# LaurenYTaylor/jsrl-CORL

Measured on AMD Instinct MI355X. Metric: IQL gradient-steps/sec at batch=256 (D4RL obs/act dims), higher is better.
Workload: dtype f32; 1 GPU; IQL step on synthetic buffer (obs=17, act=6, 1000000 rows), batch=256 per GPU; global_batch=256, parallelism=single, prepare_rehearsal_steps=1111

## Files before the change

### jsrl-corl_amd/csrc/iqlhip.hip

```cpp
#include "iqlhip_kernels.h"
#include "iqlhip_lb_kernels.h"

#include <dlfcn.h>

#include <time.h>

#include <algorithm>
#include <cstdarg>
#include <cstdio>
#include <cstdlib>
#include <cstring>
#include <string>
#include <type_traits>
#include <vector>

#define GRAPH_STEPS IQLHIP_GRAPH_STEPS
static const int kChunkSizes[] = {GRAPH_STEPS, 16, 4, 2, 1};

static thread_local std::string g_err;

static int fail(int code, const char* fmt, ...) {
  char buf[512];
  va_list ap;
  va_start(ap, fmt);
// ... 221 lines not shown
}

extern "C" int64_t iqlhip_row_stride(int32_t S, int32_t A) { return up(2 * (int64_t)S + A + 2, 4); }

static int xld_host(int k0) { int k0p = (k0 + 3) & ~3; return ((k0p + 29) / 32) * 32 + 2; }

extern "C" int iqlhip_destroy(iqlhip_ctx* c);
extern "C" int iqlhip_xch_shutdown(iqlhip_ctx* c);

static int create_impl(iqlhip_ctx* c, const iqlhip_dims* dims, const iqlhip_hyper* hyper, int device) {
  c->dims = *dims;
  c->hyper = *hyper;
  c->device = device;
  iqlhip_arena_layout(dims, &c->L);
  const int MB = dims->max_batch, A = dims->action_dim;
  c->n_chunk_max = (MB + CHUNK_ROWS - 1) / CHUNK_ROWS;
  c->n_rt_max = (MB + RT_ROWS - 1) / RT_ROWS;
  c->sc.max_batch = MB;
  auto dalloc = [&](float** p, size_t nfloat) -> hipError_t {
    hipError_t e = hipMalloc((void**)p, nfloat * sizeof(float));
    if (e != hipSuccess) return e;
    return hipMemset(*p, 0, nfloat * sizeof(float));
  };
  HIPCHK(dalloc(&c->sc.h0, (size_t)4 * MB * HID));
  HIPCHK(dalloc(&c->sc.h1, (size_t)4 * MB * HID));
  HIPCHK(dalloc(&c->sc.heads, (size_t)MB * HEAD_LD + (size_t)NSPLIT * MB * A));
  c->row_ld = iqlhip_row_stride(dims->state_dim, A);
  HIPCHK(dalloc(&c->xb, (size_t)MB * c->row_ld));
  HIPCHK(dalloc(&c->xb2, (size_t)MB * c->row_ld));
  HIPCHK(hipHostMalloc((void**)&c->losses_host, 4 * sizeof(float), hipHostMallocDefault));
  HIPCHK(hipHostMalloc((void**)&c->on_row_pin, (size_t)c->row_ld * sizeof(float), hipHostMallocDefault));
  HIPCHK(hipHostMalloc((void**)&c->on_idx_pin, (size_t)MB * sizeof(long long), hipHostMallocDefault));
  HIPCHK(hipHostMalloc((void**)&c->on_loss_pin, 4 * sizeof(float), hipHostMallocDefault));
  HIPCHK(hipHostMalloc((void**)&c->done_pin, 8 * sizeof(unsigned long long), hipHostMallocDefault));
  memset(c->done_pin, 0, 8 * sizeof(unsigned long long));
  HIPCHK(hipHostMalloc((void**)&c->on_act_pin, (size_t)(IQLHIP_MAX_INPUT + IQLHIP_MAX_ACTION) * sizeof(float), hipHostMallocDefault));
  c->act_cap = std::max(MB, IQLHIP_ACT_ROWS);
  HIPCHK(dalloc(&c->xb_act, (size_t)c->act_cap * c->row_ld));
  HIPCHK(dalloc(&c->heads_act, (size_t)c->act_cap * A * NSPLIT));
  HIPCHK(hipMalloc((void**)&c->drop_bits, (size_t)4 * MB * 8 * sizeof(unsigned)));
  HIPCHK(hipMemset(c->drop_bits, 0xFF, (size_t)4 * MB * 8 * sizeof(unsigned)));
  HIPCHK(dalloc(&c->sc.slab_a, (size_t)c->n_chunk_max * c->L.n_params));
  size_t sb = 0;
  for (int n = 0; n < 4; ++n) {
    c->sc.slab_b_off[n] = (long long)sb;
    sb += (size_t)c->n_rt_max * ((size_t)HID * c->L.net[n].k_in + HID);
  }
  HIPCHK(dalloc(&c->sc.slab_b, sb));
// ... 1688 lines not shown
    if (which == 1 || which == 3 || which == 4 || which == 5) launch_bwd(c, p, st);
    if (which == 2 || which == 3) launch_upd(c, u, st);
  }
  c->lb_bwd_part = 0;
  HIPCHK(hipEventRecord(e1, st));
  HIPCHK(hipEventSynchronize(e1));
  float ms = 0.f;
  HIPCHK(hipEventElapsedTime(&ms, e0, e1));
  *avg_us = ms * 1e3f / repeat;
  (void)hipEventDestroy(e0);
  (void)hipEventDestroy(e1);
  return IQLHIP_OK;
}

extern "C" int iqlhip_debug_read(iqlhip_ctx* c, const char* name, float* host_out, int64_t max_floats, int64_t* n_out,
                                 void* stream) {
  if (!c || !name || !host_out) return fail(IQLHIP_EINVAL, "NULL argument");
  hipStream_t st = (hipStream_t)stream;
  const float* src = nullptr;
  int64_t n = 0;
  const int MB = c->dims.max_batch;
  if (!strcmp(name, "h0")) { src = c->sc.h0; n = (int64_t)4 * MB * HID; }
  else if (!strcmp(name, "h1")) { src = c->sc.h1; n = (int64_t)4 * MB * HID; }
  else if (!strcmp(name, "heads")) { src = c->sc.heads; n = (int64_t)MB * HEAD_LD + (int64_t)NSPLIT * MB * c->dims.action_dim; }
  else if (!strcmp(name, "loss_parts")) { src = c->sc.loss_parts; n = 4 * 64; }
  else if (!strcmp(name, "drop_bits")) { src = (const float*)c->drop_bits; n = (int64_t)2 * MB * 8; }
  else if (!strcmp(name, "stamps")) {
    if (!c->stamps) return fail(IQLHIP_EINVAL, "library built without -DIQL_STAMPS");
    src = (const float*)c->stamps; n = 4096 * 16 * 2;
  }
  else if (!strcmp(name, "grads")) {
    return fail(IQLHIP_EINVAL, "use iqlhip_forward_backward to obtain the flat gradient");
  } else return fail(IQLHIP_EINVAL, "unknown scratch array '%s'", name);
  if (n > max_floats) n = max_floats;
  HIPCHK(hipMemcpyAsync(host_out, src, (size_t)n * sizeof(float), hipMemcpyDeviceToHost, st));
  HIPCHK(hipStreamSynchronize(st));
  if (n_out) *n_out = n;
  return IQLHIP_OK;
}


template <class T> struct Section { size_t off = 0; };
struct Staging {
  char* dev = nullptr;
  char* pin = nullptr;
  size_t bytes = 0;
// ... 538 lines not shown
```

### jsrl-corl_amd/csrc/iqlhip_bwd_body.inc

```
  RT_ENTRY();
  const int bid = blockIdx.x;
  const int x = bid & 7;
  const int h_S = (int)(q_dims & 255u), h_A = (int)((q_dims >> 8) & 63u), h_pol = (int)((q_dims >> 14) & 1u);
  const int h_ld = (int)(q_ldB & 1023u), h_rows = (int)(q_ldB >> 10);
  const int h_MB = (int)(q_mbc & 0xFFFFu), n_chunk = (int)(q_mbc >> 16);
  const int n_rt = (int)(q_rts & 1023u), h_spb = (int)(q_rts >> 10);
  unsigned kpf[8] = {0, 0, 0, 0, 0, 0, 0, 0};
  if constexpr (!MULTI && KPF) {
    const unsigned long long ka = (unsigned long long)(uintptr_t)__builtin_amdgcn_kernarg_segment_ptr();
    constexpr unsigned KA_P = 56;
    const unsigned o_net = KA_P + (unsigned)offsetof(StepParams, net) + (unsigned)sizeof(NetPtrs) * (unsigned)(x & 3);
    const unsigned o_go = KA_P + (unsigned)offsetof(StepParams, go) + (unsigned)sizeof(NetGrad) * (unsigned)(x & 3);
    const unsigned o_t0 = (KA_P + (unsigned)offsetof(StepParams, log_std)) & ~63u;
    static_assert(KA_P + sizeof(StepParams) - ((KA_P + offsetof(StepParams, log_std)) & ~(size_t)63) <= 256, "kernel-argument tail: more than 4 lines");
    unsigned d0, d1, d2, d3, d4, d5, d6, d7;
    asm volatile(
        "s_load_dword %0, %8, %9\n\ts_load_dword %1, %8, %10\n\ts_load_dword %2, %8, %11\n\t"
        "s_load_dword %3, %8, %12\n\ts_load_dword %4, %8, %13\n\ts_load_dword %5, %8, %14\n\t"
        "s_load_dword %6, %8, %15\n\ts_load_dword %7, %8, %16"
        : "=&s"(d0), "=&s"(d1), "=&s"(d2), "=&s"(d3), "=&s"(d4), "=&s"(d5), "=&s"(d6), "=&s"(d7)
        : "s"(ka), "s"(o_net), "s"(o_net + (unsigned)sizeof(NetPtrs) - 4u), "s"(o_go), "s"(o_go + (unsigned)sizeof(NetGrad) - 4u),
          "s"(o_t0), "s"(o_t0 + 64u), "s"(o_t0 + 128u), "s"(o_t0 + 192u));
    kpf[0] = d0; kpf[1] = d1; kpf[2] = d2; kpf[3] = d3; kpf[4] = d4; kpf[5] = d5; kpf[6] = d6; kpf[7] = d7;
  }
// ... 10 lines not shown
      const int j = q * 6 + (x - (x >> 2));
      if (net == IQLHIP_NET_PI || j >= n_don) return;
      net = IQLHIP_NET_PI;
      local_ = n_a + n_b - n_don + j;
    } else {
      local_ -= 2 * n_e;
      if (net == IQLHIP_NET_PI && local_ >= n_a + n_b - n_don) return;
    }
  }
  const int tid = threadIdx.x, lane = tid & 63, wave = tid >> 6;
  const int l15 = lane & 15, g = lane >> 4;
  const int B = h_rows;
  const int MB = h_MB;
  const ArenaOff ao = arena_off(net, h_S, h_A, h_pol == IQLHIP_POLICY_GAUSSIAN);

  const NetPtrs np = p.net[net];
  const NetGrad go = p.go[net];
  const int D = ao.d;
  const int Dp = (D + 15) & ~15;
  const int DYLD = Dp + 4;
  const float* w2 = q_params + ao.w2;
  const float* H1g = BF16 ? (const float*)((const __bf16*)q_h1 + net * MB * HID) : q_h1 + net * MB * HID;
  const float* H0g = BF16 ? (const float*)((const __bf16*)q_h0 + net * MB * HID) : q_h0 + net * MB * HID;
#define PIN_REST()                                                                                                          \
  do {                                                                                                                      \
    float* sa_ = p.sc.slab_a; float* sb_ = p.sc.slab_b;                                                                     \
    const long long sbo_ = p.sc.slab_b_off[net], npar_ = p.n_params;                                                        \
    PIN_P(np.w1); PIN_P(sa_); PIN_P(sb_);                                                                                   \
    PIN_S(sbo_); PIN_S(npar_); PIN_S(go.w1); PIN_S(go.b1); PIN_S(go.w2); PIN_S(go.b2); PIN_S(go.log_std);                   \
    PIN_S(p.inv_batch); PIN_S(p.hy.iql_tau); PIN_S(p.hy.beta); PIN_S(p.hy.discount); PIN_S(p.hy.exp_adv_max);               \
    if constexpr (!MULTI && KPF)                                                                                            \
      asm volatile("s_waitcnt lgkmcnt(0)" ::"s"(kpf[0]), "s"(kpf[1]), "s"(kpf[2]), "s"(kpf[3]), "s"(kpf[4]), "s"(kpf[5]),   \
                   "s"(kpf[6]), "s"(kpf[7]));                                                                               \
  } while (0)
  if (local_ >= n_a + n_b) return;
  const int local = MULTI ? ((local_ < n_b) ? n_a + local_ : local_ - n_b) : local_;

  extern __shared__ __attribute__((aligned(16))) float smem[];
  STAMP_BASE(p, 2048 * 16);
  STAMP(p, 0);

  if (local < n_a) {
    const int c = local >> 5;
    const int jt = (local >> 2) & 7;
    const int it = local & 3;
    const int j0 = jt * 32, i0 = it * 64;
    const int cbase = c * CHUNK_ROWS;
    float* red = smem;
    const int DYA = Dp + 4;
    float* dYs = red + 4 * 32 * T64_LD;
    float* dLs = dYs + CHUNK_ROWS * DYA;
    float* W2s = dLs + CHUNK_ROWS * DYA;
    float* rsm = W2s + 32 * 32;
    float* wS = rsm + 64;
    const bool designated = (jt == 0 && it == 2);
    const bool loss_block = (jt == 1 && it == 2);
    const bool do_db1 = (it == 0);
    const bool do_dw2 = (D == 1) ? (it == 0) : (it == 1 || it == 3);
    const int tb_own = (it == 3) ? 1 : 0;
    const bool extras = do_db1 || do_dw2;

    const int prow = cbase + tid;
    RowIn in;
    const float lsr = pi_ls_issue_hot(q_params + ao.log_std, q_xb, h_pol, h_A);
    const bool is_pi = (net == IQLHIP_NET_PI);
    row_issue_hot(q_heads, q_xb, h_ld, h_S, h_A, BROW(prow), in);
    const int r8 = tid >> 3, sub = tid & 7;
    const f32x4* hpb = (const f32x4*)(q_heads + MB * HEAD_LD);
    const float* hpf = q_heads + MB * HEAD_LD;
    const float* xbp = q_xb;
    f32x4 php[8];
    float pac[8];
    if (is_pi) {
      const unsigned dd0 = (unsigned)min(sub, h_A - 1);
      const unsigned uA = (unsigned)h_A, uld = (unsigned)h_ld, uS = (unsigned)h_S;
#pragma unroll
      for (int cc = 0; cc < 8; ++cc) {
        const unsigned rowc = (unsigned)BROW(cbase + r8 + 32 * cc);
        php[cc] = *(const f32x4*)(hpf + 4u * (rowc * uA + dd0));
        pac[cc] = xbp[rowc * uld + uS + dd0];
      }
    }
    float w2pre[4];
#pragma unroll
    for (int q = 0; q < 4; ++q) {
      const int ec = min(tid + 256 * q, D * 32 - 1);
      w2pre[q] = w2[(unsigned)((ec >> 5) * HID + j0 + (ec & 31))];
    }
#define AROW(ks) (64 * wave + 16 * ((ks) >> 2) + 4 * g + ((ks) & 3))
    typename Frag2<BF16>::type hh[16];
    typename Frag4<BF16>::type bb[16];
#define HB_LOAD(k0_, k1_)                                                                               \
    _Pragma("unroll") for (int ks = (k0_); ks < (k1_); ++ks) {                                          \
      const unsigned row = (unsigned)BROW(cbase + AROW(ks));                                            \
      hh[ks] = ld2<BF16>(H1g, row * (unsigned)HID + (unsigned)(j0 + 2 * l15));                          \
      bb[ks] = ld4<BF16>(H0g, row * (unsigned)HID + (unsigned)(i0 + 4 * l15));                          \
    }
    HB_LOAD(0, 4);
    PIN_REST();
    float* slab = p.sc.slab_a + (long long)c * p.n_params;
    const float dscale = (net == IQLHIP_NET_PI && p.drop_bits != nullptr) ? p.drop_scale : 1.f;
    STAMP(p, 10);
    {
      const int row = prow;
#pragma unroll
      for (int q = 0; q < 4; ++q) {
        const int e = tid + 256 * q;
        if (e < Dp * 32) W2s[e] = (e < D * 32) ? w2pre[q] : 0.f;
      }
      float lossA = 0.f, lossB = 0.f;
      const PiConst pc = pi_consts_hot(p, h_pol, net, lsr);
      if (!is_pi) {
        float* dyrow = dYs + tid * DYA;
        for (int dd = 0; dd < Dp; ++dd) dyrow[dd] = 0.f;
        if (row < B) row_finish(p, net, in, dyrow, lossA, lossB);
      } else {
        float wrow = 0.f;
        if (row < B) {
// ... 124 lines not shown
      __syncthreads();
      if (tid < D) {
        float u[32], w[32];
#pragma unroll
        for (int k = 0; k < 32; ++k) { u[k] = red[k * 16 + tid]; w[k] = red[k * 16 + 8 + tid]; }
#pragma unroll
        for (int st = 16; st > 0; st >>= 1) {
#pragma unroll
          for (int k = 0; k < 16; ++k) if (k < st) { u[k] += u[k + st]; w[k] += w[k + st]; }
        }
        const float ts = u[0], tl = w[0];
        slab[go.b2 + tid] = ts;
        if (gls) {
          const bool inside = (lsr >= p.hy.log_std_min) && (lsr <= p.hy.log_std_max);
          slab[go.log_std + tid] = inside ? tl * p.inv_batch : 0.f;
        }
      }
    }
    STAMP(p, 2);

    float av[16][2];
    float db1a[2] = {0.f, 0.f};
    float dw2a[2] = {0.f, 0.f};
    if (D == 1) {
      const float w2a = W2s[2 * l15], w2b = W2s[2 * l15 + 1];
#pragma unroll
      for (int ks = 0; ks < 16; ++ks) {
        const float dy = dYs[AROW(ks) * DYA];
        av[ks][0] = ((float)hh[ks][0] > 0.f) ? dy * w2a * dscale : 0.f;
        av[ks][1] = ((float)hh[ks][1] > 0.f) ? dy * w2b * dscale : 0.f;
        if (do_dw2) {
          dw2a[0] = fmaf(dy, (float)hh[ks][0], dw2a[0]);
          dw2a[1] = fmaf(dy, (float)hh[ks][1], dw2a[1]);
        }
      }
    } else {
      f32x4 pre[4][2];
#pragma unroll
      for (int t = 0; t < 4; ++t) { pre[t][0] = (f32x4){0.f, 0.f, 0.f, 0.f}; pre[t][1] = pre[t][0]; }
      if (D <= 8) dh1_mfma<2>(pre, dYs, W2s, DYA, wave, g, l15);
      else if (D <= 16) dh1_mfma<4>(pre, dYs, W2s, DYA, wave, g, l15);
      else dh1_mfma<8>(pre, dYs, W2s, DYA, wave, g, l15);
#pragma unroll
      for (int ks = 0; ks < 16; ++ks) {
        av[ks][0] = ((float)hh[ks][0] > 0.f) ? pre[ks >> 2][0][ks & 3] * dscale : 0.f;
        av[ks][1] = ((float)hh[ks][1] > 0.f) ? pre[ks >> 2][1][ks & 3] * dscale : 0.f;
      }
    }
    if (do_db1) {
#pragma unroll
      for (int ks = 0; ks < 16; ++ks) { db1a[0] += av[ks][0]; db1a[1] += av[ks][1]; }
    }

    f32x4 acc[2][4];
#pragma unroll
    for (int i = 0; i < 2; ++i)
#pragma unroll
      for (int j = 0; j < 4; ++j) acc[i][j] = (f32x4){0.f, 0.f, 0.f, 0.f};
    if constexpr (BF16) {
#pragma unroll
      for (int q = 0; q < 2; ++q) {
        bf16x8 A[2], Bv[4];
#pragma unroll
        for (int ta = 0; ta < 2; ++ta) {
          float t8[8];
#pragma unroll
          for (int e = 0; e < 8; ++e) t8[e] = av[8 * q + e][ta];
          A[ta] = pack8s(t8);
        }
#pragma unroll
        for (int tb = 0; tb < 4; ++tb) {
// ... 6 lines not shown
          for (int tb = 0; tb < 4; ++tb) acc[ta][tb] = MFMA_BF16(A[ta], Bv[tb], acc[ta][tb]);
      }
    } else {
#pragma unroll
      for (int ks = 0; ks < 16; ++ks) {
#pragma unroll
        for (int ta = 0; ta < 2; ++ta)
#pragma unroll
          for (int tb = 0; tb < 4; ++tb) acc[ta][tb] = MFMA16(av[ks][ta], bb[ks][tb], acc[ta][tb]);
      }
    }
    f32x4 acc2[2][2];
#pragma unroll
    for (int i = 0; i < 2; ++i)
#pragma unroll
      for (int j = 0; j < 2; ++j) acc2[i][j] = (f32x4){0.f, 0.f, 0.f, 0.f};
    const int ndt = Dp >> 4;
    if (do_dw2 && D > 1) {
      float ad[16];
#pragma unroll
      for (int ks = 0; ks < 16; ++ks) ad[ks] = dYs[AROW(ks) * DYA + l15];
      float hsel[16];
#pragma unroll
      for (int ks = 0; ks < 16; ++ks) hsel[ks] = tb_own ? (float)hh[ks][1] : (float)hh[ks][0];
#pragma unroll
      for (int ks = 0; ks < 16; ++ks) acc2[0][0] = MFMA16(ad[ks], hsel[ks], acc2[0][0]);
      if (ndt > 1) {
#pragma unroll
        for (int ks = 0; ks < 16; ++ks) ad[ks] = dYs[AROW(ks) * DYA + 16 + l15];
#pragma unroll
        for (int ks = 0; ks < 16; ++ks) acc2[1][0] = MFMA16(ad[ks], hsel[ks], acc2[1][0]);
      }
    }
    STAMP(p, 3);

    float* exA = dLs;
    float* exB = dLs + 1024;
    {
      float* myred = red + wave * 32 * T64_LD;
#pragma unroll
      for (int ta = 0; ta < 2; ++ta)
#pragma unroll
        for (int reg = 0; reg < 4; ++reg) {
          const int jl = 2 * (4 * g + reg) + ta;
          f32x4 v = (f32x4){acc[ta][0][reg], acc[ta][1][reg], acc[ta][2][reg], acc[ta][3][reg]};
          *(f32x4*)(myred + jl * T64_LD + 4 * l15) = v;
        }
// ... 23 lines not shown
        for (int w = 1; w < 4; ++w) s += *(const f32x4*)(red + w * 32 * T64_LD + jl * T64_LD + 4 * i4);
        *(f32x4*)(gw1 + (j0 + jl) * HID + i0 + 4 * i4) = s;
      }
    }
    if (extras) {
      const int e_lo = do_db1 ? 0 : 32;
      const int e_hi = do_dw2 ? (1 + D) * 32 : 32;
      for (int e = tid + e_lo; e < e_hi; e += 256) {
        const int rr = e >> 5, jj = e & 31;
        float s;
        if (rr == 0 || D == 1) {
          float wsum[4];
#pragma unroll
          for (int w = 0; w < 4; ++w) {
            const float* a = exA + (w * 4) * 64 + rr * 32 + jj;
            wsum[w] = (a[0] + a[64]) + (a[128] + a[192]);
          }
          s = (wsum[0] + wsum[1]) + (wsum[2] + wsum[3]);
        } else {
          const float* b = exB + (rr - 1) * 32 + jj;
          s = (b[0] + b[1024]) + (b[2048] + b[3072]);
        }
        if (rr == 0) { if (do_db1) slab[go.b1 + j0 + jj] = s; }
        else if (do_dw2 && (D == 1 || (jj & 1) == tb_own)) slab[go.w2 + (rr - 1) * HID + j0 + jj] = s;
      }
    }
    STAMP(p, 4);
    RT_STAMP(p, 14, rt_entry_);
    RT_STAMP(p, 15, iql_realtime());
    return;
  }
#undef AROW

  {
    const int lb = local - n_a;
    const int rt = lb >> (2 - bsl2);
    int i0 = ((lb & ((4 >> bsl2) - 1)) << bsl2) * 64;
    const int row0 = rt * RT_ROWS;
    const int k0 = ao.k0;
    const int ld = h_ld;
    const int xoff = 0;
    const float* w1 = np.w1;

    float* dH1s = smem;
    __bf16* dH1b = (__bf16*)smem;
    float* red = dH1s + RT_ROWS * H0_LD;
    float* dH0s = red + 4 * 32 * T64_LD;
// ... 15 lines not shown
      const float* hsb = q_heads;
      const unsigned oh = (unsigned)prow8 * (unsigned)HEAD_LD;
      ph[0] = *(const f32x4*)(hsb + (oh + 4u)); ph[1] = *(const f32x4*)(hsb + (oh + 8u)); ph[2] = *(const f32x4*)(hsb + (oh + 12u));
      const float* arow = q_xb + (unsigned)(prow8 * h_ld + h_S);
      const f32x4* hp = (const f32x4*)(q_heads + MB * HEAD_LD + (unsigned)(prow8 * h_A * NSPLIT));
#pragma unroll
      for (int c = 0; c < 4; ++c) {
        php[c] = (f32x4){0.f, 0.f, 0.f, 0.f};
        pac[c] = 0.f;
        if (c == 0 || 8 * c < h_A) {
          const int dd = min(psub + 8 * c, h_A - 1);
          php[c] = hp[dd];
          pac[c] = arow[dd];
        }
      }
    }
    const int j4 = tid & 63;
    const f32x4 w2v = *(const f32x4*)(w2 + 4 * j4);
    f32x4 w2v8[8];
    if (D > 1) {
#pragma unroll
      for (int j = 0; j < 8; ++j) w2v8[j] = *(const f32x4*)(w2 + min(j, D - 1) * HID + 4 * j4);
    }
    typename Frag4<BF16>::type h1v[8];
#define H1V_LOAD(q0_, q1_)                                                                              \
    _Pragma("unroll") for (int q = (q0_); q < (q1_); ++q) {                                             \
      const int f = tid + 256 * q;                                                                      \
      const unsigned row = (unsigned)BROW(row0 + (f >> 6));           \
      h1v[q] = ld4<BF16>(H1g, row * (unsigned)HID + (unsigned)(4 * (f & 63)));                          \
    }
    H1V_LOAD(0, 4);
    constexpr bool FULLB = BF16 && MULTI;
    typename Frag4<BF16>::type bw[FULLB ? 64 : 16];
    typename Frag4<BF16>::type h0v[2];
    const int n_x = RT_ROWS * ld / 4;
    const int x_last = B * ld / 4 - 1;
    PIN_REST();
    const float dscale = (net == IQLHIP_NET_PI && p.drop_bits != nullptr) ? p.drop_scale : 1.f;

    const PiConst pc = pi_consts_hot(p, h_pol, net, lsr);
    if (net == IQLHIP_NET_PI) {
      const float tq = fminf(sum4(ph[1]), sum4(ph[2]));
      const float u = tq - sum4(ph[0]);
      const float w = fminf(expf(p.hy.beta * u), p.hy.exp_adv_max);
      const bool rvalid = (row0 + prl) < B;
      const bool gauss = (h_pol == IQLHIP_POLICY_GAUSSIAN);
#pragma unroll
      for (int c = 0; c < 4; ++c) {
        const int dd = psub + 8 * c;
        if (dd < Dp) {
          float dy = 0.f;
          const int ddc = min(dd, h_A - 1);
          const float ivar = __shfl(pc.ivar, ddc);
          if (rvalid && dd < h_A) {
            const float mu = tanh_via_exp(sum4(php[c]));
            const float diff = pac[c] - mu;
            const float dmu = gauss ? (-(w * diff) * ivar) * p.inv_batch : (-2.f * w * diff) * p.inv_batch;
            dy = dmu * (1.f - mu * mu);
          }
          dYs[prl * DYLD + dd] = dy;
        }
      }
    } else if (tid < RT_ROWS) {
      const int row = row0 + tid;
      float la, lbv;
      float* dyrow = dYs + tid * DYLD;
      for (int dd = 0; dd < Dp; ++dd) dyrow[dd] = 0.f;
      if (row < B) row_finish(p, net, in, dyrow, la, lbv);
    }
    __builtin_amdgcn_sched_barrier(0);
    H1V_LOAD(4, 8);
#undef H1V_LOAD
#pragma unroll
    for (int q = 0; q < 2; ++q) {
      const int f = tid + 256 * q;
      const unsigned row = (unsigned)BROW(row0 + (f >> 4));
      h0v[q] = ld4<BF16>(H0g, row * (unsigned)HID + (unsigned)(i0 + 4 * (f & 15)));
    }
    __builtin_amdgcn_sched_barrier(0);
    __syncthreads();
    STAMP(p, 5);
#define BWB_ROW(ks_) (FULLB ? (32 * ((ks_) >> 3) + 8 * g + ((ks_) & 7)) : (BF16 ? (64 * wave + 32 * ((ks_) >> 3) + 8 * g + ((ks_) & 7)) : (64 * wave + 4 * (ks_) + g)))
#define BWB_COL (FULLB ? (64 * wave + 4 * l15) : (i0 + 4 * l15))
#define BWB_LOAD(ks_) bw[ks_] = ld4<BF16>(w1, (unsigned)(BWB_ROW(ks_) * HID + BWB_COL))

    if (D > 8) {
      f32x4 sacc[8];
#pragma unroll
      for (int q = 0; q < 8; ++q) sacc[q] = (f32x4){0.f, 0.f, 0.f, 0.f};
      f32x4 wv[8], wn[8];
#pragma unroll
      for (int j = 0; j < 8; ++j) wv[j] = w2v8[j];
      for (int d0 = 0; d0 < D; d0 += 8) {
        const bool more = (d0 + 8 < D);
        if (more) {
#pragma unroll
          for (int j = 0; j < 8; ++j) wn[j] = *(const f32x4*)(w2 + min(d0 + 8 + j, D - 1) * HID + 4 * j4);
        }
#pragma unroll
        for (int q = 0; q < 8; ++q) {
          const int rl = (tid + 256 * q) >> 6;
          const f32x4 ya = *(const f32x4*)(dYs + rl * DYLD + d0), yb = *(const f32x4*)(dYs + rl * DYLD + d0 + 4);
#pragma unroll
          for (int j = 0; j < 4; ++j) sacc[q] += ya[j] * wv[j];
#pragma unroll
          for (int j = 0; j < 4; ++j) sacc[q] += yb[j] * wv[4 + j];
        }
        if (more) {
#pragma unroll
          for (int j = 0; j < 8; ++j) wv[j] = wn[j];
        }
      }
#pragma unroll
      for (int q = 0; q < 8; ++q) {
        const int rl = (tid + 256 * q) >> 6;
        f32x4 out;
#pragma unroll
        for (int e = 0; e < 4; ++e) out[e] = ((float)h1v[q][e] > 0.f) ? sacc[q][e] * dscale : 0.f;
        if constexpr (BF16) {
          bf16x4 ob_;
#pragma unroll
          for (int e = 0; e < 4; ++e) ob_[e] = (__bf16)out[e];
          *(bf16x4*)(dH1b + rl * H0B_LD + 4 * j4) = ob_;
        } else {
          *(f32x4*)(dH1s + rl * H0_LD + 4 * j4) = out;
        }
        if constexpr (FULLB) {
#pragma unroll
          for (int e = 0; e < 8; ++e) BWB_LOAD(8 * q + e);
        } else {
          BWB_LOAD(2 * q);
          BWB_LOAD(2 * q + 1);
        }
      }
    } else {
      f32x4 sq[8];
      if (D == 1) {
        float dy1[8];
#pragma unroll
        for (int q = 0; q < 8; ++q) dy1[q] = dYs[((tid + 256 * q) >> 6) * DYLD];
#pragma unroll
// ... 5 lines not shown
#pragma unroll
          for (int qq = 0; qq < 4; ++qq) {
            const int rl = (tid + 256 * (4 * hq + qq)) >> 6;
            ya[qq] = *(const f32x4*)(dYs + rl * DYLD);
            yb[qq] = *(const f32x4*)(dYs + rl * DYLD + 4);
          }
#pragma unroll
          for (int qq = 0; qq < 4; ++qq) {
            f32x4 s = ya[qq][0] * w2v8[0];
#pragma unroll
            for (int j = 1; j < 4; ++j) s += ya[qq][j] * w2v8[j];
#pragma unroll
            for (int j = 0; j < 4; ++j) s += yb[qq][j] * w2v8[4 + j];
            sq[4 * hq + qq] = s;
          }
        }
      }
#pragma unroll
      for (int q = 0; q < 8; ++q) {
        const int rl = (tid + 256 * q) >> 6;
        const f32x4 s = sq[q];
        f32x4 out;
#pragma unroll
        for (int e = 0; e < 4; ++e) out[e] = ((float)h1v[q][e] > 0.f) ? s[e] * dscale : 0.f;
        if constexpr (BF16) {
          bf16x4 ob_;
#pragma unroll
          for (int e = 0; e < 4; ++e) ob_[e] = (__bf16)out[e];
          *(bf16x4*)(dH1b + rl * H0B_LD + 4 * j4) = ob_;
        } else {
          *(f32x4*)(dH1s + rl * H0_LD + 4 * j4) = out;
        }
        if constexpr (FULLB) {
#pragma unroll
          for (int e = 0; e < 8; ++e) BWB_LOAD(8 * q + e);
        } else {
          BWB_LOAD(2 * q);
          BWB_LOAD(2 * q + 1);
        }
      }
    }
    __syncthreads();
    STAMP(p, 6);
    if constexpr (FULLB) {
      typename Frag4<true>::type hm[2][4];
#pragma unroll
      for (int rtl = 0; rtl < 2; ++rtl)
// ... 74 lines not shown
            if (kc0 + 3 < k0) {
              *(f32x4u*)(slabB + (unsigned)(il * k0 + kc0)) = r4;
            } else {
#pragma unroll
              for (int reg = 0; reg < 4; ++reg) {
                const int kc = kc0 + reg;
                if (kc < k0) slabB[(unsigned)(il * k0 + kc)] = r4[reg];
                else if (kc == k0) dstB[il] = r4[reg];
              }
            }
          }
        }
      }
      STAMP(p, 9);
      RT_STAMP(p, 14, rt_entry_);
      RT_STAMP(p, 15, iql_realtime());
      return;
    }
    f32x4 xr[XR_MAX_F4];
    xr_load(xr, q_xb, row0 * ld / 4, n_x, x_last);

    for (int itn = 0;; ++itn) {
    const bool more = MULTI && (itn + 1 < (1 << bsl2));
    typename Frag4<BF16>::type h0n[2] = {h0v[0], h0v[1]};

    {
      f32x4 acc[2][4];
#pragma unroll
      for (int i = 0; i < 2; ++i)
#pragma unroll
        for (int j = 0; j < 4; ++j) acc[i][j] = (f32x4){0.f, 0.f, 0.f, 0.f};
      if constexpr (BF16) {
#pragma unroll
        for (int q = 0; q < 2; ++q) {
          const bf16x8 A0 = *(const bf16x8*)(dH1b + l15 * H0B_LD + 64 * wave + 32 * q + 8 * g);
          const bf16x8 A1 = *(const bf16x8*)(dH1b + (16 + l15) * H0B_LD + 64 * wave + 32 * q + 8 * g);
#pragma unroll
          for (int tb = 0; tb < 4; ++tb) {
            bf16x8 Bv;
#pragma unroll
            for (int e = 0; e < 8; ++e) Bv[e] = bw[8 * q + e][tb];
            acc[0][tb] = MFMA_BF16(A0, Bv, acc[0][tb]);
            acc[1][tb] = MFMA_BF16(A1, Bv, acc[1][tb]);
          }
          if (more) {
#pragma unroll
            for (int ks = 8 * q; ks < 8 * q + 8; ++ks)
// ... 3 lines not shown
      } else {
#pragma unroll
        for (int ks = 0; ks < 16; ++ks) {
          const int kk = 64 * wave + 4 * ks + g;
          const float a0 = dH1s[l15 * H0_LD + kk];
          const float a1 = dH1s[(16 + l15) * H0_LD + kk];
#pragma unroll
          for (int tb = 0; tb < 4; ++tb) {
            acc[0][tb] = MFMA16(a0, bw[ks][tb], acc[0][tb]);
            acc[1][tb] = MFMA16(a1, bw[ks][tb], acc[1][tb]);
          }
          if ((ks & 3) == 3 && more) {
#pragma unroll
            for (int k2 = ks - 3; k2 <= ks; ++k2)
              bw[k2] = ld4<BF16>(w1, (unsigned)((64 * wave + 4 * k2 + g) * HID + i0 + 64 + 4 * l15));
          }
        }
      }
      if (more) {
#pragma unroll
        for (int q = 0; q < 2; ++q) {
          const int f = tid + 256 * q;
          const unsigned row = (unsigned)BROW(row0 + (f >> 4));
          h0n[q] = ld4<BF16>(H0g, row * (unsigned)HID + (unsigned)(i0 + 64 + 4 * (f & 15)));
        }
      }
      float* myred = red + wave * 32 * T64_LD;
#pragma unroll
      for (int rtile = 0; rtile < 2; ++rtile)
#pragma unroll
        for (int reg = 0; reg < 4; ++reg) {
          const int rl = 16 * rtile + 4 * g + reg;
          f32x4 v = (f32x4){acc[rtile][0][reg], acc[rtile][1][reg], acc[rtile][2][reg], acc[rtile][3][reg]};
          *(f32x4*)(myred + rl * T64_LD + 4 * l15) = v;
        }
    }
    if (itn == 0) xr_store(xr, Xr, n_x);
    __syncthreads();
    STAMP(p, 7);
#pragma unroll
    for (int q = 0; q < 2; ++q) {
      const int f = tid + 256 * q;
      const int rl = f >> 4, i4 = f & 15;
      f32x4 s = *(const f32x4*)(red + rl * T64_LD + 4 * i4);
#pragma unroll
      for (int w = 1; w < 4; ++w) s += *(const f32x4*)(red + w * 32 * T64_LD + rl * T64_LD + 4 * i4);
      f32x4 out;
#pragma unroll
      for (int e = 0; e < 4; ++e) out[e] = ((float)h0v[q][e] > 0.f) ? s[e] * dscale : 0.f;
      *(f32x4*)(dH0s + rl * T64_LD + 4 * i4) = out;
    }
    __syncthreads();

    STAMP(p, 8);
    float* slabB = p.sc.slab_b + p.sc.slab_b_off[net] + rt * (HID * k0 + HID);
    {
      int k0_ = k0;
      if constexpr (MULTI) asm volatile("" : "+s"(k0_));
      const int k0 = k0_;
      const int k1 = k0 + 1;
      const int nct = (k1 + 15) >> 4;
      f32x4 acc[9];
#pragma unroll
      for (int ct = 0; ct < 9; ++ct) acc[ct] = (f32x4){0.f, 0.f, 0.f, 0.f};
      float bv[8];
#pragma unroll
      for (int ks = 0; ks < 8; ++ks) bv[ks] = dH0s[(4 * ks + g) * T64_LD + 16 * wave + l15];
#pragma unroll
      for (int ct = 0; ct < 9; ++ct) {
        if (ct < nct) {
          const int kc = 16 * ct + l15;
          const int kcc = min(kc, k0 - 1);
// ... 49 lines not shown
```

### jsrl-corl_amd/csrc/iqlhip_fwd_body.inc

```
  RT_ENTRY();
  const int bid = blockIdx.x;
  const int fx = bid & 7, fh = fx >> 2, fr = bid >> 3;
  constexpr unsigned FWD_PAIR_A = 0x6541u, FWD_PAIR_B = 0x7320u;
  const int inst = ONE ? p.only_inst : (int)((((fr & 1) ? FWD_PAIR_B : FWD_PAIR_A) >> (4 * (fx & 3))) & 7u);
  if (inst >= 7) {
    if (p.g_work) idle_block_work(p.g_work, (fr >> 1) * 2 + fh, (int)(gridDim.x >> 3));
    return;
  }
  const int spb_l2 = MULTI ? (p.spb_l2 & 3) : 0;
  const int spb = 1 << spb_l2;
  int ns, rt;
  if (ONE) {
    ns = bid & (NSPLIT - 1);
    rt = bid >> 2;
  } else if (spb_l2 == 0) {
    ns = 2 * ((fr >> 1) & 1) + fh;
    rt = fr >> 2;
  } else if (spb_l2 == 1) {
    ns = 2 * fh;
    rt = fr >> 1;
  } else {
    ns = 0;
    rt = 2 * (fr >> 1) + fh;
    if (rt * RT_ROWS >= p.rows) return;
// ... 265 lines not shown
          *(f32x4*)(H0s + (rtile * 16 + l15) * H0_LD + wave * 64 + ct * 16 + 4 * g) = h;
        }
      }
    }
  }
  STAMP(p, 7);
  __syncthreads();
  STAMP(p, 2);

  for (int it = 0;; ++it) {
  const bool more = MULTI && (it + 1 < spb);
  f32x4 bias1n = bias1;
  if (more) {
#pragma unroll
    for (int q = 0; q < 2; ++q) {
      const int e = min(tid + 256 * q, D * 16 - 1);
      w2pre[q] = *(const f32x4*)(np.w2 + (unsigned)((e >> 4) * HID + (ns + 1) * 64 + 4 * (e & 15)));
    }
    bias1n = *(const f32x4*)(np.b1 + (unsigned)((ns + 1) * 64 + wave * 16 + 4 * g));
  }
  if (slot >= 0) {
    const int rl = tid >> 3;
    const int row = row0 + rl;
    if (row < B) {
#pragma unroll
      for (int j = 0; j < 2; ++j) {
        const int col = ns * 64 + 4 * ((tid & 7) + 8 * j);
        if constexpr (BF16)
          *(bf16x4*)((__bf16*)h0g + (unsigned)((slot * MB + row) * HID + col)) = *(const bf16x4*)(H0b + rl * H0B_LD + col);
        else
          *(f32x4*)(h0g + (unsigned)((slot * MB + row) * HID + col)) = *(const f32x4*)(H0s + rl * H0_LD + col);
      }
    }
  }

  if (it == 0) STAMP(p, 8);
  {
    f32x4 acc0 = (f32x4){0.f, 0.f, 0.f, 0.f}, acc1 = acc0;
    if constexpr (BF16) {
      bf16x8 b0[8], b1[8];
#pragma unroll
      for (int j = 0; j < 8; ++j) {
        b0[j] = *(const bf16x8*)(H0b + l15 * H0B_LD + 32 * j + 8 * g);
        b1[j] = *(const bf16x8*)(H0b + (16 + l15) * H0B_LD + 32 * j + 8 * g);
      }
#pragma unroll
      for (int j = 0; j < 8; ++j) {
        acc0 = MFMA_BF16(bwb[j], b0[j], acc0);
        acc1 = MFMA_BF16(bwb[j], b1[j], acc1);
        if ((j & 1) && more) {
          bwb[j - 1] = BWB_AT(n1 + 64, j - 1);
          bwb[j] = BWB_AT(n1 + 64, j);
        }
      }
// ... 23 lines not shown
    }
    if (drop) {
      const int word = ns * 2 + (wave >> 1), sh = (wave & 1) * 16 + 4 * g;
      const unsigned ba = Mk[256 + l15 * 8 + word] >> sh, bb_ = Mk[256 + (16 + l15) * 8 + word] >> sh;
#pragma unroll
      for (int reg = 0; reg < 4; ++reg) {
        h0[reg] = ((ba >> reg) & 1u) ? h0[reg] * p.drop_scale : 0.f;
        h1[reg] = ((bb_ >> reg) & 1u) ? h1[reg] * p.drop_scale : 0.f;
      }
    }
    *(f32x4*)(H1s + l15 * T64_LD + wave * 16 + 4 * g) = h0;
    *(f32x4*)(H1s + (16 + l15) * T64_LD + wave * 16 + 4 * g) = h1;
  }
  if (it == 0) STAMP(p, 10);
  __syncthreads();
  if (it == 0) STAMP(p, 11);
  STAMP(p, 3);
  if (more) n1 += 64;

  {
    const int rl = tid >> 3;
    const int row = row0 + rl;
    const int sub = tid & 7;
    if (slot >= 0 && row < B) {
#pragma unroll
      for (int j = 0; j < 2; ++j) {
        const int cl = 4 * (sub + 8 * j);
        st4<BF16>(h1g, (unsigned)((slot * MB + row) * HID + ns * 64 + cl), *(const f32x4*)(H1s + rl * T64_LD + cl));
      }
    }
    const f32x4 ha = *(const f32x4*)(H1s + rl * T64_LD + 4 * sub);
    const f32x4 hb = *(const f32x4*)(H1s + rl * T64_LD + 32 + 4 * sub);
    if (D == 1) {
      const f32x4 wa = *(const f32x4*)(W2s + 4 * sub);
      const f32x4 wb = *(const f32x4*)(W2s + 32 + 4 * sub);
      float acc = 0.f;
#pragma unroll
      for (int e = 0; e < 4; ++e) acc = fmaf(ha[e], wa[e], acc);
#pragma unroll
      for (int e = 0; e < 4; ++e) acc = fmaf(hb[e], wb[e], acc);
      acc += __shfl_xor(acc, 1);
      acc += __shfl_xor(acc, 2);
      acc += __shfl_xor(acc, 4);
      if (ns == 0) acc += W2s[Dp * W2_LD];
      if (sub == 0 && row < B) {
        if (inst < 6) headsg[row * HEAD_LD + inst * NSPLIT + ns] = acc;
        else headsg[MB * HEAD_LD + row * NSPLIT + ns] = acc;
      }
    } else {
      if (16 * (wave >> 1) < Dp) {
        const int i = wave & 1, nt = wave >> 1;
// ... 35 lines not shown
```

### jsrl-corl_amd/csrc/iqlhip_kernels.h

```cpp
#pragma once
#include <hip/hip_runtime.h>
#include <stdint.h>
#include "iqlhip.h"

typedef float f32x4 __attribute__((ext_vector_type(4)));
typedef float f32x2 __attribute__((ext_vector_type(2)));
typedef float f32x4u __attribute__((ext_vector_type(4), aligned(4)));

#define HID 256
#define RT_ROWS 32
#define CHUNK_ROWS 256
#define H0_LD 260
#define H0B_LD 264
#define T64_LD 68
#define NSPLIT 4
#define HEAD_LD 24
#define W0_LDS_MAX_K 64
#define W0_DMA_MAX_K 96
#define W2_LD 68

#define MFMA16(a, b, c) __builtin_amdgcn_mfma_f32_16x16x4f32((a), (b), (c), 0, 0, 0)

typedef __bf16 bf16x8 __attribute__((ext_vector_type(8)));
#define MFMA_BF16(a, b, c) __builtin_amdgcn_mfma_f32_16x16x32_bf16((a), (b), (c), 0, 0, 0)
// ... 16 lines not shown
template <bool BF16> struct Frag2 { typedef f32x2 type; };
template <> struct Frag2<true> { typedef bf16x2 type; };
template <bool BF16> __device__ __forceinline__ typename Frag4<BF16>::type ld4(const float* base, unsigned off) {
  if constexpr (BF16) return *(const bf16x4*)((const __bf16*)base + off);
  else return *(const f32x4*)(base + off);
}
template <bool BF16> __device__ __forceinline__ typename Frag2<BF16>::type ld2(const float* base, unsigned off) {
  if constexpr (BF16) return *(const bf16x2*)((const __bf16*)base + off);
  else return *(const f32x2*)(base + off);
}
template <bool BF16> __device__ __forceinline__ void st4(float* base, unsigned off, const f32x4 v) {
  if constexpr (BF16) {
    bf16x4 r;
#pragma unroll
    for (int i = 0; i < 4; ++i) r[i] = (__bf16)v[i];
    *(bf16x4*)((__bf16*)base + off) = r;
  } else {
    *(f32x4*)(base + off) = v;
  }
}
__device__ __forceinline__ bf16x8 cat8(const bf16x4 lo, const bf16x4 hi) {
  return __builtin_shufflevector(lo, hi, 0, 1, 2, 3, 4, 5, 6, 7);
}

struct DevScratch {
  float* h0;
  float* h1;
  float* heads;
  float* slab_a;
  float* slab_b;
  float* loss_parts;
  float* losses;
  long long slab_b_off[4];
  int max_batch;
};

#ifdef IQL_STAMPS
__device__ __forceinline__ unsigned long long iql_memtime() {
  unsigned long long t;
  __builtin_amdgcn_sched_barrier(0);
  asm volatile("s_memtime %0\n\ts_waitcnt lgkmcnt(0)" : "=s"(t) :: "memory");
  __builtin_amdgcn_sched_barrier(0);
  return t;
}
#define STAMP(p, i)                                                                        \
  do {                                                                                     \
// ... 1091 lines not shown
```

Measured before the change: 52220 steps/s.

## Store packed ReLU activation bitmasks and read them in backward instead of activations

The forward pass in f32 mode now also writes a packed bitmask of which hidden activations are positive, with 8 words per row, built with DPP OR-reductions. The backward kernel reads these bits for ReLU gating and keeps full activation loads only where the value itself is needed (dW2). This cuts global memory traffic for the h0/h1 re-reads in backward. In exchange it adds extra stores and cross-lane work in forward, changes the dW2 work split for the f32 D==1 case, and adds more code paths to get right.

```diff
diff --git a/jsrl-corl_amd/csrc/iqlhip.hip b/jsrl-corl_amd/csrc/iqlhip.hip
--- a/jsrl-corl_amd/csrc/iqlhip.hip
+++ b/jsrl-corl_amd/csrc/iqlhip.hip
@@ -267,8 +267,8 @@
     if (e != hipSuccess) return e;
     return hipMemset(*p, 0, nfloat * sizeof(float));
   };
-  HIPCHK(dalloc(&c->sc.h0, (size_t)4 * MB * HID));
-  HIPCHK(dalloc(&c->sc.h1, (size_t)4 * MB * HID));
+  HIPCHK(dalloc(&c->sc.h0, (size_t)4 * MB * HID + (size_t)4 * MB * 8));
+  HIPCHK(dalloc(&c->sc.h1, (size_t)4 * MB * HID + (size_t)4 * MB * 8));
   HIPCHK(dalloc(&c->sc.heads, (size_t)MB * HEAD_LD + (size_t)NSPLIT * MB * A));
   c->row_ld = iqlhip_row_stride(dims->state_dim, A);
   HIPCHK(dalloc(&c->xb, (size_t)MB * c->row_ld));
@@ -2003,6 +2003,8 @@
   const int MB = c->dims.max_batch;
   if (!strcmp(name, "h0")) { src = c->sc.h0; n = (int64_t)4 * MB * HID; }
   else if (!strcmp(name, "h1")) { src = c->sc.h1; n = (int64_t)4 * MB * HID; }
+  else if (!strcmp(name, "h0_bits")) { src = c->sc.h0 + (size_t)4 * MB * HID; n = (int64_t)4 * MB * 8; }
+  else if (!strcmp(name, "h1_bits")) { src = c->sc.h1 + (size_t)4 * MB * HID; n = (int64_t)4 * MB * 8; }
   else if (!strcmp(name, "heads")) { src = c->sc.heads; n = (int64_t)MB * HEAD_LD + (int64_t)NSPLIT * MB * c->dims.action_dim; }
   else if (!strcmp(name, "loss_parts")) { src = c->sc.loss_parts; n = 4 * 64; }
   else if (!strcmp(name, "drop_bits")) { src = (const float*)c->drop_bits; n = (int64_t)2 * MB * 8; }
diff --git a/jsrl-corl_amd/csrc/iqlhip_bwd_body.inc b/jsrl-corl_amd/csrc/iqlhip_bwd_body.inc
--- a/jsrl-corl_amd/csrc/iqlhip_bwd_body.inc
+++ b/jsrl-corl_amd/csrc/iqlhip_bwd_body.inc
@@ -56,6 +56,8 @@
   const float* w2 = q_params + ao.w2;
   const float* H1g = BF16 ? (const float*)((const __bf16*)q_h1 + net * MB * HID) : q_h1 + net * MB * HID;
   const float* H0g = BF16 ? (const float*)((const __bf16*)q_h0 + net * MB * HID) : q_h0 + net * MB * HID;
+  const unsigned* H1m = relu_bits(q_h1, MB) + net * MB * 8;
+  const unsigned* H0m = relu_bits(q_h0, MB) + net * MB * 8;
 #define PIN_REST()                                                                                                          \
   do {                                                                                                                      \
     float* sa_ = p.sc.slab_a; float* sb_ = p.sc.slab_b;                                                                     \
@@ -90,7 +92,7 @@
     const bool designated = (jt == 0 && it == 2);
     const bool loss_block = (jt == 1 && it == 2);
     const bool do_db1 = (it == 0);
-    const bool do_dw2 = (D == 1) ? (it == 0) : (it == 1 || it == 3);
+    const bool do_dw2 = (BF16 && D == 1) ? (it == 0) : (it == 1 || it == 3);
     const int tb_own = (it == 3) ? 1 : 0;
     const bool extras = do_db1 || do_dw2;
 
@@ -122,12 +124,17 @@
       w2pre[q] = w2[(unsigned)((ec >> 5) * HID + j0 + (ec & 31))];
     }
 #define AROW(ks) (64 * wave + 16 * ((ks) >> 2) + 4 * g + ((ks) & 3))
-    typename Frag2<BF16>::type hh[16];
+    typename Frag2<BF16>::type hh[BF16 ? 16 : 1];
+    float hv[BF16 ? 1 : 16];
+    unsigned hw = 0;
+    const unsigned hv_sel = do_dw2 ? ~0u : 0u;
+    if constexpr (!BF16) hw = H1m[(unsigned)BROW(cbase + 64 * wave + lane) * 8u + (unsigned)jt];
     typename Frag4<BF16>::type bb[16];
 #define HB_LOAD(k0_, k1_)                                                                               \
     _Pragma("unroll") for (int ks = (k0_); ks < (k1_); ++ks) {                                          \
       const unsigned row = (unsigned)BROW(cbase + AROW(ks));                                            \
-      hh[ks] = ld2<BF16>(H1g, row * (unsigned)HID + (unsigned)(j0 + 2 * l15));                          \
+      if constexpr (BF16) hh[ks] = ld2<BF16>(H1g, row * (unsigned)HID + (unsigned)(j0 + 2 * l15));      \
+      else hv[ks] = H1g[(row * (unsigned)HID + (unsigned)(j0 + 2 * l15 + tb_own)) & hv_sel];            \
       bb[ks] = ld4<BF16>(H0g, row * (unsigned)HID + (unsigned)(i0 + 4 * l15));                          \
     }
     HB_LOAD(0, 4);
@@ -298,18 +305,30 @@
     float av[16][2];
     float db1a[2] = {0.f, 0.f};
     float dw2a[2] = {0.f, 0.f};
+    unsigned mk[BF16 ? 1 : 16];
+    if constexpr (!BF16) {
+#pragma unroll
+      for (int ks = 0; ks < 16; ++ks) mk[ks] = (unsigned)__shfl((int)hw, 16 * (ks >> 2) + 4 * g + (ks & 3)) >> (2 * l15);
+    }
+#define H1_ON(ks_, ta_) (BF16 ? ((float)hh[BF16 ? (ks_) : 0][ta_] > 0.f) : (((mk[BF16 ? 0 : (ks_)] >> (ta_)) & 1u) != 0u))
     if (D == 1) {
       const float w2a = W2s[2 * l15], w2b = W2s[2 * l15 + 1];
+      float dw2s = 0.f;
 #pragma unroll
       for (int ks = 0; ks < 16; ++ks) {
         const float dy = dYs[AROW(ks) * DYA];
-        av[ks][0] = ((float)hh[ks][0] > 0.f) ? dy * w2a * dscale : 0.f;
-        av[ks][1] = ((float)hh[ks][1] > 0.f) ? dy * w2b * dscale : 0.f;
+        av[ks][0] = H1_ON(ks, 0) ? dy * w2a * dscale : 0.f;
+        av[ks][1] = H1_ON(ks, 1) ? dy * w2b * dscale : 0.f;
         if (do_dw2) {
-          dw2a[0] = fmaf(dy, (float)hh[ks][0], dw2a[0]);
-          dw2a[1] = fmaf(dy, (float)hh[ks][1], dw2a[1]);
-        }
-      }
+          if constexpr (BF16) {
+            dw2a[0] = fmaf(dy, (float)hh[BF16 ? ks : 0][0], dw2a[0]);
+            dw2a[1] = fmaf(dy, (float)hh[BF16 ? ks : 0][1], dw2a[1]);
+          } else {
+            dw2s = fmaf(dy, hv[BF16 ? 0 : ks], dw2s);
+          }
+        }
+      }
+      if constexpr (!BF16) { dw2a[0] = tb_own ? 0.f : dw2s; dw2a[1] = tb_own ? dw2s : 0.f; }
     } else {
       f32x4 pre[4][2];
 #pragma unroll
@@ -319,10 +338,11 @@
       else dh1_mfma<8>(pre, dYs, W2s, DYA, wave, g, l15);
 #pragma unroll
       for (int ks = 0; ks < 16; ++ks) {
-        av[ks][0] = ((float)hh[ks][0] > 0.f) ? pre[ks >> 2][0][ks & 3] * dscale : 0.f;
-        av[ks][1] = ((float)hh[ks][1] > 0.f) ? pre[ks >> 2][1][ks & 3] * dscale : 0.f;
-      }
-    }
+        av[ks][0] = H1_ON(ks, 0) ? pre[ks >> 2][0][ks & 3] * dscale : 0.f;
+        av[ks][1] = H1_ON(ks, 1) ? pre[ks >> 2][1][ks & 3] * dscale : 0.f;
+      }
+    }
+#undef H1_ON
     if (do_db1) {
 #pragma unroll
       for (int ks = 0; ks < 16; ++ks) { db1a[0] += av[ks][0]; db1a[1] += av[ks][1]; }
@@ -375,7 +395,10 @@
       for (int ks = 0; ks < 16; ++ks) ad[ks] = dYs[AROW(ks) * DYA + l15];
       float hsel[16];
 #pragma unroll
-      for (int ks = 0; ks < 16; ++ks) hsel[ks] = tb_own ? (float)hh[ks][1] : (float)hh[ks][0];
+      for (int ks = 0; ks < 16; ++ks) {
+        if constexpr (BF16) hsel[ks] = tb_own ? (float)hh[BF16 ? ks : 0][1] : (float)hh[BF16 ? ks : 0][0];
+        else hsel[ks] = hv[BF16 ? 0 : ks];
+      }
 #pragma unroll
       for (int ks = 0; ks < 16; ++ks) acc2[0][0] = MFMA16(ad[ks], hsel[ks], acc2[0][0]);
       if (ndt > 1) {
@@ -445,7 +468,7 @@
           s = (b[0] + b[1024]) + (b[2048] + b[3072]);
         }
         if (rr == 0) { if (do_db1) slab[go.b1 + j0 + jj] = s; }
-        else if (do_dw2 && (D == 1 || (jj & 1) == tb_own)) slab[go.w2 + (rr - 1) * HID + j0 + jj] = s;
+        else if (do_dw2 && ((BF16 && D == 1) || (jj & 1) == tb_own)) slab[go.w2 + (rr - 1) * HID + j0 + jj] = s;
       }
     }
     STAMP(p, 4);
@@ -507,17 +530,19 @@
 #pragma unroll
       for (int j = 0; j < 8; ++j) w2v8[j] = *(const f32x4*)(w2 + min(j, D - 1) * HID + 4 * j4);
     }
-    typename Frag4<BF16>::type h1v[8];
+    typename Mask4<BF16>::type h1v[8];
+    const int msh = 4 * (tid & 7);
 #define H1V_LOAD(q0_, q1_)                                                                              \
     _Pragma("unroll") for (int q = (q0_); q < (q1_); ++q) {                                             \
       const int f = tid + 256 * q;                                                                      \
       const unsigned row = (unsigned)BROW(row0 + (f >> 6));           \
-      h1v[q] = ld4<BF16>(H1g, row * (unsigned)HID + (unsigned)(4 * (f & 63)));                          \
+      if constexpr (BF16) h1v[q] = ld4<BF16>(H1g, row * (unsigned)HID + (unsigned)(4 * (f & 63)));      \
+      else h1v[q] = H1m[row * 8u + (unsigned)((tid & 63) >> 3)];                                        \
     }
     H1V_LOAD(0, 4);
     constexpr bool FULLB = BF16 && MULTI;
     typename Frag4<BF16>::type bw[FULLB ? 64 : 16];
-    typename Frag4<BF16>::type h0v[2];
+    typename Mask4<BF16>::type h0v[2];
     const int n_x = RT_ROWS * ld / 4;
     const int x_last = B * ld / 4 - 1;
     PIN_REST();
@@ -560,7 +585,8 @@
     for (int q = 0; q < 2; ++q) {
       const int f = tid + 256 * q;
       const unsigned row = (unsigned)BROW(row0 + (f >> 4));
-      h0v[q] = ld4<BF16>(H0g, row * (unsigned)HID + (unsigned)(i0 + 4 * (f & 15)));
+      if constexpr (BF16) h0v[q] = ld4<BF16>(H0g, row * (unsigned)HID + (unsigned)(i0 + 4 * (f & 15)));
+      else h0v[q] = H0m[row * 8u + (unsigned)((i0 >> 5) + ((tid & 15) >> 3))];
     }
     __builtin_amdgcn_sched_barrier(0);
     __syncthreads();
@@ -601,7 +627,7 @@
         const int rl = (tid + 256 * q) >> 6;
         f32x4 out;
 #pragma unroll
-        for (int e = 0; e < 4; ++e) out[e] = ((float)h1v[q][e] > 0.f) ? sacc[q][e] * dscale : 0.f;
+        for (int e = 0; e < 4; ++e) out[e] = relu_on(h1v[q], e, msh) ? sacc[q][e] * dscale : 0.f;
         if constexpr (BF16) {
           bf16x4 ob_;
 #pragma unroll
@@ -653,7 +679,7 @@
         const f32x4 s = sq[q];
         f32x4 out;
 #pragma unroll
-        for (int e = 0; e < 4; ++e) out[e] = ((float)h1v[q][e] > 0.f) ? s[e] * dscale : 0.f;
+        for (int e = 0; e < 4; ++e) out[e] = relu_on(h1v[q], e, msh) ? s[e] * dscale : 0.f;
         if constexpr (BF16) {
           bf16x4 ob_;
 #pragma unroll
@@ -774,7 +800,7 @@
 
     for (int itn = 0;; ++itn) {
     const bool more = MULTI && (itn + 1 < (1 << bsl2));
-    typename Frag4<BF16>::type h0n[2] = {h0v[0], h0v[1]};
+    typename Mask4<BF16>::type h0n[2] = {h0v[0], h0v[1]};
 
     {
       f32x4 acc[2][4];
@@ -824,7 +850,8 @@
         for (int q = 0; q < 2; ++q) {
           const int f = tid + 256 * q;
           const unsigned row = (unsigned)BROW(row0 + (f >> 4));
-          h0n[q] = ld4<BF16>(H0g, row * (unsigned)HID + (unsigned)(i0 + 64 + 4 * (f & 15)));
+          if constexpr (BF16) h0n[q] = ld4<BF16>(H0g, row * (unsigned)HID + (unsigned)(i0 + 64 + 4 * (f & 15)));
+          else h0n[q] = H0m[row * 8u + (unsigned)(((i0 + 64) >> 5) + ((tid & 15) >> 3))];
         }
       }
       float* myred = red + wave * 32 * T64_LD;
@@ -849,7 +876,7 @@
       for (int w = 1; w < 4; ++w) s += *(const f32x4*)(red + w * 32 * T64_LD + rl * T64_LD + 4 * i4);
       f32x4 out;
 #pragma unroll
-      for (int e = 0; e < 4; ++e) out[e] = ((float)h0v[q][e] > 0.f) ? s[e] * dscale : 0.f;
+      for (int e = 0; e < 4; ++e) out[e] = relu_on(h0v[q], e, msh) ? s[e] * dscale : 0.f;
       *(f32x4*)(dH0s + rl * T64_LD + 4 * i4) = out;
     }
     __syncthreads();
diff --git a/jsrl-corl_amd/csrc/iqlhip_fwd_body.inc b/jsrl-corl_amd/csrc/iqlhip_fwd_body.inc
--- a/jsrl-corl_amd/csrc/iqlhip_fwd_body.inc
+++ b/jsrl-corl_amd/csrc/iqlhip_fwd_body.inc
@@ -311,14 +311,24 @@
   if (slot >= 0) {
     const int rl = tid >> 3;
     const int row = row0 + rl;
-    if (row < B) {
-#pragma unroll
-      for (int j = 0; j < 2; ++j) {
-        const int col = ns * 64 + 4 * ((tid & 7) + 8 * j);
-        if constexpr (BF16)
+    if constexpr (BF16) {
+      if (row < B) {
+#pragma unroll
+        for (int j = 0; j < 2; ++j) {
+          const int col = ns * 64 + 4 * ((tid & 7) + 8 * j);
           *(bf16x4*)((__bf16*)h0g + (unsigned)((slot * MB + row) * HID + col)) = *(const bf16x4*)(H0b + rl * H0B_LD + col);
-        else
-          *(f32x4*)(h0g + (unsigned)((slot * MB + row) * HID + col)) = *(const f32x4*)(H0s + rl * H0_LD + col);
+        }
+      }
+    } else {
+      f32x4 v[2];
+#pragma unroll
+      for (int j = 0; j < 2; ++j) v[j] = *(const f32x4*)(H0s + rl * H0_LD + ns * 64 + 4 * ((tid & 7) + 8 * j));
+      const u32x2 wd = relu_words8(v, tid & 7);
+      if (row < B) {
+#pragma unroll
+        for (int j = 0; j < 2; ++j)
+          *(f32x4*)(h0g + (unsigned)((slot * MB + row) * HID + ns * 64 + 4 * ((tid & 7) + 8 * j))) = v[j];
+        if ((tid & 7) == 0) *(u32x2*)(relu_bits(h0g, MB) + (unsigned)((slot * MB + row) * 8 + 2 * ns)) = wd;
       }
     }
   }
@@ -388,11 +398,23 @@
     const int rl = tid >> 3;
     const int row = row0 + rl;
     const int sub = tid & 7;
-    if (slot >= 0 && row < B) {
-#pragma unroll
-      for (int j = 0; j < 2; ++j) {
-        const int cl = 4 * (sub + 8 * j);
-        st4<BF16>(h1g, (unsigned)((slot * MB + row) * HID + ns * 64 + cl), *(const f32x4*)(H1s + rl * T64_LD + cl));
+    if constexpr (BF16) {
+      if (slot >= 0 && row < B) {
+#pragma unroll
+        for (int j = 0; j < 2; ++j) {
+          const int cl = 4 * (sub + 8 * j);
+          st4<BF16>(h1g, (unsigned)((slot * MB + row) * HID + ns * 64 + cl), *(const f32x4*)(H1s + rl * T64_LD + cl));
+        }
+      }
+    } else if (slot >= 0) {
+      f32x4 v[2];
+#pragma unroll
+      for (int j = 0; j < 2; ++j) v[j] = *(const f32x4*)(H1s + rl * T64_LD + 4 * (sub + 8 * j));
+      const u32x2 wd = relu_words8(v, sub);
+      if (row < B) {
+#pragma unroll
+        for (int j = 0; j < 2; ++j) *(f32x4*)(h1g + (unsigned)((slot * MB + row) * HID + ns * 64 + 4 * (sub + 8 * j))) = v[j];
+        if (sub == 0) *(u32x2*)(relu_bits(h1g, MB) + (unsigned)((slot * MB + row) * 8 + 2 * ns)) = wd;
       }
     }
     const f32x4 ha = *(const f32x4*)(H1s + rl * T64_LD + 4 * sub);
diff --git a/jsrl-corl_amd/csrc/iqlhip_kernels.h b/jsrl-corl_amd/csrc/iqlhip_kernels.h
--- a/jsrl-corl_amd/csrc/iqlhip_kernels.h
+++ b/jsrl-corl_amd/csrc/iqlhip_kernels.h
@@ -62,6 +62,31 @@
 __device__ __forceinline__ bf16x8 cat8(const bf16x4 lo, const bf16x4 hi) {
   return __builtin_shufflevector(lo, hi, 0, 1, 2, 3, 4, 5, 6, 7);
 }
+
+typedef unsigned u32x2 __attribute__((ext_vector_type(2)));
+__device__ __forceinline__ unsigned* relu_bits(float* h, int MB) { return (unsigned*)(h + (size_t)4 * MB * HID); }
+__device__ __forceinline__ const unsigned* relu_bits(const float* h, int MB) { return (const unsigned*)(h + (size_t)4 * MB * HID); }
+__device__ __forceinline__ unsigned or8_dpp(unsigned v) {
+  v |= (unsigned)__builtin_amdgcn_update_dpp(0, (int)v, 0xB1, 0xF, 0xF, true);
+  v |= (unsigned)__builtin_amdgcn_update_dpp(0, (int)v, 0x4E, 0xF, 0xF, true);
+  v |= (unsigned)__builtin_amdgcn_update_dpp(0, (int)v, 0x141, 0xF, 0xF, true);
+  return v;
+}
+__device__ __forceinline__ u32x2 relu_words8(const f32x4 (&v)[2], int sub) {
+  u32x2 r;
+#pragma unroll
+  for (int j = 0; j < 2; ++j) {
+    unsigned nib = 0;
+#pragma unroll
+    for (int e = 0; e < 4; ++e) nib |= (v[j][e] > 0.f) ? (1u << e) : 0u;
+    r[j] = or8_dpp(nib << (4 * sub));
+  }
+  return r;
+}
+__device__ __forceinline__ bool relu_on(unsigned w, int e, int sh) { return ((w >> (sh + e)) & 1u) != 0u; }
+__device__ __forceinline__ bool relu_on(const bf16x4 h, int e, int) { return (float)h[e] > 0.f; }
+template <bool BF16> struct Mask4 { typedef unsigned type; };
+template <> struct Mask4<true> { typedef bf16x4 type; };
 
 struct DevScratch {
   float* h0;
```

Measured after the change: 50420 steps/s. 0.965x the previous value.
